# zhangxinsong-nlp/XFM

Hardware: AMD Instinct MI355X
Metric: image-text pairs/sec fwd+bwd, XFM-base 224px/30tok (higher is better)
Workload: dtype bf16; 1 GPU; Pretrain.py full multimodal step (ITC+ITM+MLM+MIM), XFM-base, synthetic 224px images + 30-token captions, random init; units_per_gpu=64, global_batch=64, dropout=True, ordered_reductions=True, grad_allreduce=False, parallelism=dp1, image_res=224

## Files before the change

### xfm_amd/csrc/gemm.hip

```cpp
#include "common.h"

enum { EPI_BF16 = 0, EPI_F32 = 1, EPI_GELU = 2, EPI_DGELU = 3, EPI_F32_ACC = 4 };

#define XFM_FENCE() asm volatile("" ::: "memory")
#define XFM_BAR()                    \
  do {                               \
    XFM_FENCE();                     \
    __builtin_amdgcn_s_barrier();    \
    XFM_FENCE();                     \
  } while (0)


struct GemmNT {
  const bf16* A; long lda;
  const bf16* B; long ldb;
  void* C; long ldc;
  const float* bias;
  bf16* aux; long ldaux;
  int M, N, K;
  int group_m;
  int k_splits;
  long split_stride;
#ifdef XFM_DIAG
  long long* dbg;
// ... 48 lines not shown
      for (int i = 0; i < 4; ++i) {
        v[i] = acc[mt][2 * np][i] + bv[i];
        v[4 + i] = acc[mt][2 * np + 1][i] + bv[4 + i];
      }
      const bool full = (nb + 8 <= g.N) && vec_c;
      if (EPI == EPI_F32 || EPI == EPI_F32_ACC) {
        float* cp = reinterpret_cast<float*>(g.C) + (long)m * g.ldc + nb;
        if (EPI == EPI_F32 && g.k_splits > 1) {
          cp += (long)blockIdx.y * g.split_stride;
        }
        if (EPI == EPI_F32_ACC && g.k_splits > 1) {
          for (int i = 0; i < 8; ++i)
            if (nb + i < g.N) atomicAdd(cp + i, v[i] - (blockIdx.y == 0 ? 0.f : bv[i]));
          continue;
        }
        if (EPI == EPI_F32_ACC) {
          for (int i = 0; i < 8; ++i)
            if (nb + i < g.N) v[i] += cp[i];
        }
        if (full) {
          *reinterpret_cast<f32x4*>(cp) = f32x4{v[0], v[1], v[2], v[3]};
          *reinterpret_cast<f32x4*>(cp + 4) = f32x4{v[4], v[5], v[6], v[7]};
        } else {
          for (int i = 0; i < 8; ++i)
            if (nb + i < g.N) cp[i] = v[i];
        }
      } else {
        bf16* cp = reinterpret_cast<bf16*>(g.C) + (long)m * g.ldc + nb;
        bf16x8 o;
        if (EPI == EPI_GELU) {
          bf16* ap = g.aux + (long)m * g.ldaux + nb;
          bf16x8 dact;
#pragma unroll
          for (int i = 0; i < 8; ++i) {
            const float x = bf2f(f2bf(v[i]));
            float cdf, pdf;
            gelu_parts(x, cdf, pdf);
            o[i] = f2bf(x * cdf);
            dact[i] = f2bf(fmaf(x, pdf, cdf));
          }
          if (full) *reinterpret_cast<bf16x8*>(ap) = dact;
          else
            for (int i = 0; i < 8; ++i)
              if (nb + i < g.N) ap[i] = dact[i];
        } else if (EPI == EPI_DGELU) {
          const bf16* ap = g.aux + (long)m * g.ldaux + nb;
          if (full && vec_aux) {
            const bf16x8 dact = pre_all[np][mt];
#pragma unroll
            for (int i = 0; i < 8; ++i) o[i] = f2bf(v[i] * bf2f(dact[i]));
          } else {
            for (int i = 0; i < 8; ++i) o[i] = (nb + i < g.N) ? f2bf(v[i] * bf2f(ap[i])) : f2bf(0.f);
          }
        } else {
#pragma unroll
          for (int i = 0; i < 8; ++i) o[i] = f2bf(v[i]);
        }
        if (full) *reinterpret_cast<bf16x8*>(cp) = o;
        else
          for (int i = 0; i < 8; ++i)
            if (nb + i < g.N) cp[i] = o[i];
      }
    }
  }
}


template <int BM, int BN, int EPI, int NS>
__global__ __launch_bounds__(256) void gemm_nt_kernel(GemmNT g) {
  constexpr int MT = BM / 32, NT = BN / 32;
  constexpr int LOADS = (BM + BN) / 32;
  constexpr int A_BYTES = BM * 128, B_BYTES = BN * 128, STAGE = A_BYTES + B_BYTES;
  extern __shared__ __attribute__((aligned(16))) char smem[];
  const int tid = threadIdx.x, lane = tid & 63, w = tid >> 6;
  const int wm = w >> 1, wn = w & 1;
  const int lr = lane & 15, lg = lane >> 4;
  const int tiles_n = (g.N + BN - 1) / BN, tiles_m = (g.M + BM - 1) / BM;
  const int wg = xcd_remap(blockIdx.x, gridDim.x);
  int tm, tn;
  grouped_tile(wg, tiles_m, tiles_n, g.group_m, tm, tn);
  const int m0 = tm * BM, n0 = tn * BN;

  const int nk_all = g.K / 64;
  const int nk_per = (nk_all + g.k_splits - 1) / g.k_splits;
  const int kt0 = blockIdx.y * nk_per;
  const int nk = nk_all - kt0 < nk_per ? nk_all - kt0 : nk_per;
  if (nk <= 0) return;
  auto stage = [&](int buf, int kt) {
    char* sA = smem + buf * STAGE;
    char* sB = sA + A_BYTES;
    const int k0 = (kt0 + kt) * 64;
#pragma unroll
    for (int i = 0; i < BM / 32; ++i) {
      const int blk = i * 4 + w;
      const int r = blk * 8 + (lane >> 3);
      const int c = (lane & 7) ^ swz_x(r);
      int gr = m0 + r;
      gr = gr < g.M ? gr : g.M - 1;
      const bf16* src = g.A + (long)gr * g.lda + k0 + c * 8;
      __builtin_amdgcn_global_load_lds(GLB_PTR(void, src), LDS_PTR(void, sA + blk * 1024), 16, 0, 0);
    }
#pragma unroll
    for (int i = 0; i < BN / 32; ++i) {
      const int blk = i * 4 + w;
      const int r = blk * 8 + (lane >> 3);
      const int c = (lane & 7) ^ swz_w(r);
      int gr = n0 + r;
      gr = gr < g.N ? gr : g.N - 1;
      const bf16* src = g.B + (long)gr * g.ldb + k0 + c * 8;
      __builtin_amdgcn_global_load_lds(GLB_PTR(void, src), LDS_PTR(void, sB + blk * 1024), 16, 0, 0);
    }
  };

  f32x4 acc[MT][NT];
#pragma unroll
  for (int i = 0; i < MT; ++i)
#pragma unroll
    for (int j = 0; j < NT; ++j) acc[i][j] = f32x4{0.f, 0.f, 0.f, 0.f};

  int xrow[MT], wrow[NT];
#pragma unroll
  for (int mt = 0; mt < MT; ++mt) xrow[mt] = wm * (BM / 2) + mt * 16 + lr;
#pragma unroll
  for (int nt = 0; nt < NT; ++nt) wrow[nt] = wn * (BN / 2) + (nt >> 1) * 32 + 8 * (lr >> 2) + 4 * (nt & 1) + (lr & 3);

  if (NS == 2) {
    stage(0, 0);
    asm volatile("s_waitcnt vmcnt(0)" ::: "memory");
    __syncthreads();
  } else {
#pragma unroll
    for (int s0 = 0; s0 < NS - 1; ++s0)
      if (s0 < nk) stage(s0, s0);
  }
  int slot = 0;
  for (int kt = 0; kt < nk; ++kt) {
    if (NS == 2) {
      if (kt + 1 < nk) stage((kt & 1) ^ 1, kt + 1);
    } else {
      const int younger = nk - 1 - kt < NS - 2 ? nk - 1 - kt : NS - 2;
      if (younger >= 2) asm volatile("s_waitcnt vmcnt(%0)" ::"n"(2 * LOADS) : "memory");
      else if (younger == 1) asm volatile("s_waitcnt vmcnt(%0)" ::"n"(LOADS) : "memory");
      else asm volatile("s_waitcnt vmcnt(0)" ::: "memory");
      XFM_BAR();
      if (kt + NS - 1 < nk) stage(slot == 0 ? NS - 1 : slot - 1, kt + NS - 1);
    }
    const int cur = NS == 2 ? (kt & 1) : slot;
    const char* sA = smem + cur * STAGE;
    const char* sB = sA + A_BYTES;
#pragma unroll
    for (int ks = 0; ks < 2; ++ks) {
      const int c = ks * 4 + lg;
      bf16x8 xf[MT], wf[NT];
#pragma unroll
      for (int mt = 0; mt < MT; ++mt)
        xf[mt] = *reinterpret_cast<const bf16x8*>(sA + xrow[mt] * 128 + ((c ^ swz_x(xrow[mt])) << 4));
#pragma unroll
      for (int nt = 0; nt < NT; ++nt)
        wf[nt] = *reinterpret_cast<const bf16x8*>(sB + wrow[nt] * 128 + ((c ^ swz_w(wrow[nt])) << 4));
#pragma unroll
      for (int mt = 0; mt < MT; ++mt)
#pragma unroll
        for (int nt = 0; nt < NT; ++nt)
          acc[mt][nt] = __builtin_amdgcn_mfma_f32_16x16x32_bf16(wf[nt], xf[mt], acc[mt][nt], 0, 0, 0);
    }
    if (NS == 2) {
      asm volatile("s_waitcnt vmcnt(0)" ::: "memory");
      __syncthreads();
    } else {
      slot = slot == NS - 1 ? 0 : slot + 1;
    }
  }

  gemm_epilogue<MT, NT, EPI>(g, acc, m0 + wm * (BM / 2), n0 + wn * (BN / 2), lr, lg);
}

template <int EPI>
__global__ __launch_bounds__(512) void gemm_nt_ring_kernel(GemmNT g) {
  constexpr int BM = 256, BN = 128, MT = 4, NT = 4;
  constexpr int A_BYTES = BM * 128, B_BYTES = BN * 128, STAGE = A_BYTES + B_BYTES;
  extern __shared__ __attribute__((aligned(16))) char smem[];
  const int tid = threadIdx.x, lane = tid & 63, w = tid >> 6;
  const int wm = w >> 1, wn = w & 1;
  const int lr = lane & 15, lg = lane >> 4;
  const int tiles_n = (g.N + BN - 1) / BN, tiles_m = (g.M + BM - 1) / BM;
  const int wg = xcd_remap(blockIdx.x, gridDim.x);
  int tm, tn;
  grouped_tile(wg, tiles_m, tiles_n, g.group_m, tm, tn);
  const int m0 = tm * BM, n0 = tn * BN;

  auto stage = [&](int slot, int kt) {
    char* sA = smem + slot * STAGE;
    char* sB = sA + A_BYTES;
    const int k0 = kt * 64;
#pragma unroll
    for (int i = 0; i < 4; ++i) {
      const int blk = i * 8 + w;
      const int r = blk * 8 + (lane >> 3);
      const int c = (lane & 7) ^ swz_x(r);
      int gr = m0 + r;
      gr = gr < g.M ? gr : g.M - 1;
      __builtin_amdgcn_global_load_lds(GLB_PTR(void, g.A + (long)gr * g.lda + k0 + c * 8), LDS_PTR(void, sA + blk * 1024), 16, 0, 0);
    }
#pragma unroll
    for (int i = 0; i < 2; ++i) {
      const int blk = i * 8 + w;
      const int r = blk * 8 + (lane >> 3);
      const int c = (lane & 7) ^ swz_w(r);
      int gr = n0 + r;
      gr = gr < g.N ? gr : g.N - 1;
      __builtin_amdgcn_global_load_lds(GLB_PTR(void, g.B + (long)gr * g.ldb + k0 + c * 8), LDS_PTR(void, sB + blk * 1024), 16, 0, 0);
    }
  };

  f32x4 acc[MT][NT];
#pragma unroll
  for (int i = 0; i < MT; ++i)
#pragma unroll
    for (int j = 0; j < NT; ++j) acc[i][j] = f32x4{0.f, 0.f, 0.f, 0.f};
  int xrow[MT], wrow[NT];
#pragma unroll
  for (int mt = 0; mt < MT; ++mt) xrow[mt] = wm * 64 + mt * 16 + lr;
#pragma unroll
  for (int nt = 0; nt < NT; ++nt) wrow[nt] = wn * 64 + (nt >> 1) * 32 + 8 * (lr >> 2) + 4 * (nt & 1) + (lr & 3);

  const int nk = g.K / 64;
  stage(0, 0);
  if (nk > 1) stage(1, 1);
  int slot = 0;
  for (int kt = 0; kt < nk; ++kt) {
    if (kt + 1 < nk) asm volatile("s_waitcnt vmcnt(6)" ::: "memory");
    else asm volatile("s_waitcnt vmcnt(0)" ::: "memory");
    __builtin_amdgcn_s_barrier();
    if (kt + 2 < nk) stage(slot == 0 ? 2 : slot - 1, kt + 2);
    const char* sA = smem + slot * STAGE;
    const char* sB = sA + A_BYTES;
#pragma unroll
    for (int ks = 0; ks < 2; ++ks) {
      const int c = ks * 4 + lg;
      bf16x8 xf[MT], wf[NT];
#pragma unroll
      for (int mt = 0; mt < MT; ++mt)
        xf[mt] = *reinterpret_cast<const bf16x8*>(sA + xrow[mt] * 128 + ((c ^ swz_x(xrow[mt])) << 4));
#pragma unroll
      for (int nt = 0; nt < NT; ++nt)
        wf[nt] = *reinterpret_cast<const bf16x8*>(sB + wrow[nt] * 128 + ((c ^ swz_w(wrow[nt])) << 4));
#pragma unroll
      for (int mt = 0; mt < MT; ++mt)
#pragma unroll
        for (int nt = 0; nt < NT; ++nt)
          acc[mt][nt] = __builtin_amdgcn_mfma_f32_16x16x32_bf16(wf[nt], xf[mt], acc[mt][nt], 0, 0, 0);
    }
    slot = slot == 2 ? 0 : slot + 1;
  }
  gemm_epilogue<MT, NT, EPI>(g, acc, m0 + wm * 64, n0 + wn * 64, lr, lg);
}

static int launch_nt_ring(const GemmNT& g, int epi, hipStream_t st) {
  const int tiles = cdiv(g.M, 256) * cdiv(g.N, 128);
  const size_t smem = 3 * (256 + 128) * 128;
#define XFM_RING_CASE(E)                                                                                       \
  case E: {                                                                                                    \
    static bool attr_set = false;                                                                              \
    if (!attr_set) {                                                                                           \
      (void)hipFuncSetAttribute(reinterpret_cast<const void*>(gemm_nt_ring_kernel<E>),                         \
                                hipFuncAttributeMaxDynamicSharedMemorySize, (int)smem);                        \
      attr_set = true;                                                                                         \
    }                                                                                                          \
    hipLaunchKernelGGL((gemm_nt_ring_kernel<E>), dim3(tiles), dim3(512), smem, st, g);                         \
    break;                                                                                                     \
  }
  switch (epi) {
    XFM_RING_CASE(EPI_BF16)
    XFM_RING_CASE(EPI_F32)
    XFM_RING_CASE(EPI_GELU)
    XFM_RING_CASE(EPI_DGELU)
    XFM_RING_CASE(EPI_F32_ACC)
    default:
      xfm_set_error("gemm_nt: bad epilogue %d", epi);
      return XFM_E_ARG;
  }
#undef XFM_RING_CASE
  return xfm_check_launch("gemm_nt_ring");
}

template <int J>
__device__ __forceinline__ int unit_row(int u) {
  if (J == 0) return u + (u & 64);
  if (J == 3) return u + 64 + (u & 64);
  if (J == 1) return ((u >> 5) << 6) + (u & 31);
  return ((u >> 5) << 6) + 32 + (u & 31);
}


__device__ __forceinline__ void wait_younger(int y) {
  if (y >= 3) asm volatile("s_waitcnt vmcnt(6)" ::: "memory");
  else if (y == 2) asm volatile("s_waitcnt vmcnt(4)" ::: "memory");
  else if (y == 1) asm volatile("s_waitcnt vmcnt(2)" ::: "memory");
  else asm volatile("s_waitcnt vmcnt(0)" ::: "memory");
}

template <int N>
__device__ __forceinline__ void wait_vm() { asm volatile("s_waitcnt vmcnt(%0)" ::"n"(N) : "memory"); }
template <int NS, int YMAX>
__device__ __forceinline__ void wait_units(int y) {
  if (YMAX >= 5 && y == 5) wait_vm<10 + NS>();
  else if (YMAX >= 4 && y == 4) wait_vm<8 + NS>();
  else if (y >= 3) wait_vm<6 + NS>();
  else if (y == 2) wait_vm<4 + NS>();
  else if (y == 1) wait_vm<2 + NS>();
  else wait_vm<NS>();
}
constexpr int NT256_D = 5;
template <int EPI, bool PERSIST>
__global__ __launch_bounds__(512) void gemm_nt_256_kernel(GemmNT g, int tiles) {
  constexpr int BM = 256, BN = 256, MT = 8, NT = 4;
  constexpr int D = NT256_D, R = D + 3, UNIT = 128 * 128;
  constexpr int NS = !PERSIST ? 0 : EPI == EPI_GELU || EPI == EPI_F32 ? 32 : EPI == EPI_F32_ACC ? 0 : 16;
  extern __shared__ __attribute__((aligned(16))) char smem[];
  const int tid = threadIdx.x, lane = tid & 63, w = __builtin_amdgcn_readfirstlane(tid >> 6);
  const int wr = w >> 2, wc = w & 3;
  const int lr = lane & 15, lg = lane >> 4;
  const int tiles_n = (g.N + BN - 1) / BN, tiles_m = (g.M + BM - 1) / BM;
  const int nk = g.K / 64;
  const int total = 4 * nk;

  unsigned soff[4][2];
  auto tile_origin = [&](int v, int& m0, int& n0) {
    int tm, tn;
    grouped_tile(xcd_remap(v, tiles), tiles_m, tiles_n, g.group_m, tm, tn);
    m0 = tm * BM;
    n0 = tn * BN;
  };
  auto tile_offsets = [&](int m0, int n0) {
#pragma unroll
    for (int i = 0; i < 2; ++i) {
      const int u = (i * 8 + w) * 8 + (lane >> 3);
      {
        const int r = unit_row<0>(u);
        int gr = m0 + r; gr = gr < g.M ? gr : g.M - 1;
        soff[0][i] = (unsigned)gr * (unsigned)g.lda + (((lane & 7) ^ swz_x(r)) << 3);
      }
      {
        const int r = unit_row<3>(u);
        int gr = m0 + r; gr = gr < g.M ? gr : g.M - 1;
        soff[3][i] = (unsigned)gr * (unsigned)g.lda + (((lane & 7) ^ swz_x(r)) << 3);
      }
      {
        const int r = unit_row<1>(u);
        int gr = n0 + r; gr = gr < g.N ? gr : g.N - 1;
        soff[1][i] = (unsigned)gr * (unsigned)g.ldb + (((lane & 7) ^ swz_w(r)) << 3);
      }
      {
        const int r = unit_row<2>(u);
        int gr = n0 + r; gr = gr < g.N ? gr : g.N - 1;
        soff[2][i] = (unsigned)gr * (unsigned)g.ldb + (((lane & 7) ^ swz_w(r)) << 3);
      }
    }
  };
  int iss = 0;
  auto issue = [&](int s) {
    char* base = smem + iss * UNIT + w * 1024;
    iss = iss + 1 == R ? 0 : iss + 1;
    if (s >= total) return;
    const int j = s & 3;
    const bf16* src = ((j == 0 || j == 3) ? g.A : g.B) + (s >> 2) * 64;
#pragma unroll
    for (int i = 0; i < 2; ++i) {
      const unsigned so = j == 0 ? soff[0][i] : j == 1 ? soff[1][i] : j == 2 ? soff[2][i] : soff[3][i];
      const unsigned lds_addr = (unsigned)(uintptr_t)LDS_PTR(void, base) + (unsigned)(i * 8192);
      asm volatile("s_mov_b32 m0, %1\n\ts_nop 0\n\tglobal_load_lds_dwordx4 %0, off" ::"v"(src + (size_t)so), "s"(lds_addr) : "memory", "m0");
    }
  };

  f32x4 acc[MT][NT];

  const int xs = swz_x(lr);
  const int wu = 8 * (lr >> 2) + (lr & 3);
  const int ws = swz_w(wu);
  const int xbase0 = (wr * 64 + lr) * 128 + (((0 + lg) ^ xs) << 4), xbase1 = (wr * 64 + lr) * 128 + (((4 + lg) ^ xs) << 4);
  const int wbase0 = (wc * 32 + wu) * 128 + (((0 + lg) ^ ws) << 4), wbase1 = (wc * 32 + wu) * 128 + (((4 + lg) ^ ws) << 4);

  bf16x8 xa[4][2], wb0[2][2], wb1[2][2];
  auto read_x = [&](const char* slot) {
#pragma unroll
    for (int m = 0; m < 4; ++m) {
      xa[m][0] = *reinterpret_cast<const bf16x8*>(slot + xbase0 + m * 2048);
      xa[m][1] = *reinterpret_cast<const bf16x8*>(slot + xbase1 + m * 2048);
    }
  };
  auto read_w = [&](const char* slot, bf16x8 (&wb)[2][2]) {
#pragma unroll
    for (int n = 0; n < 2; ++n) {
      wb[n][0] = *reinterpret_cast<const bf16x8*>(slot + wbase0 + n * 512);
      wb[n][1] = *reinterpret_cast<const bf16x8*>(slot + wbase1 + n * 512);
    }
  };
#define XFM_QUAD(MH, NH, WB)                                                                                     \
  do {                                                                                                           \
    __builtin_amdgcn_s_setprio(1);                                                                               \
    _Pragma("unroll") for (int ks = 0; ks < 2; ++ks)                                                             \
    _Pragma("unroll") for (int m = 0; m < 4; ++m)                                                                \
    _Pragma("unroll") for (int n = 0; n < 2; ++n)                                                                \
      acc[MH * 4 + m][NH * 2 + n] =                                                                              \
          __builtin_amdgcn_mfma_f32_16x16x32_bf16(WB[n][ks], xa[m][ks], acc[MH * 4 + m][NH * 2 + n], 0, 0, 0);  \
    __builtin_amdgcn_s_setprio(0);                                                                               \
  } while (0)

  int v = blockIdx.x, m0, n0;
  tile_origin(v, m0, n0);
  tile_offsets(m0, n0);
#pragma unroll
  for (int s = 0; s < D; ++s) issue(s);
  bool stores_behind = false;

#ifdef XFM_DIAG
  int dbg_n = 0;
#endif
  while (true) {
#ifdef XFM_DIAG
    if (g.dbg != nullptr && tid == 0) {
      long long* d = g.dbg + ((long)blockIdx.x * 8 + dbg_n) * 4;
      d[0] = v; d[1] = wall_clock64();
    }
#endif
#pragma unroll
    for (int i = 0; i < MT; ++i)
#pragma unroll
      for (int j = 0; j < NT; ++j) acc[i][j] = f32x4{0.f, 0.f, 0.f, 0.f};
    {
      const int y = (total - 1 < D - 1 ? total - 1 : D - 1) - 1;
      if (NS > 0 && stores_behind) wait_units<NS, D - 2>(y);
      else wait_units<0, D - 2>(y);
    }
    XFM_BAR();
    if (wr == 1) XFM_BAR();

    int rs = 0;
    for (int kt = 0; kt < nk; ++kt) {
      const int ph = 4 * kt;
      const bool plus = NS > 0 && stores_behind && kt == 0;
      const char* s_a0 = smem + rs * UNIT;
      const char* s_b0 = smem + (rs + 1 >= R ? rs + 1 - R : rs + 1) * UNIT;
      const char* s_b1 = smem + (rs + 2 >= R ? rs + 2 - R : rs + 2) * UNIT;
      const char* s_a1 = smem + (rs + 3 >= R ? rs + 3 - R : rs + 3) * UNIT;
      rs = rs + 4 >= R ? rs + 4 - R : rs + 4;
      int last;
      issue(ph + D);
      read_x(s_a0);
      read_w(s_b0, wb0);
      last = ph + D < total ? ph + D : total - 1;
      if (plus) wait_units<NS, D - 2>(last - (ph + 2));
      else wait_units<0, D - 2>(last - (ph + 2));
      XFM_BAR();
      XFM_QUAD(0, 0, wb0);
      XFM_BAR();
      issue(ph + D + 1);
      read_w(s_b1, wb1);
      last = ph + D + 1 < total ? ph + D + 1 : total - 1;
      if (plus) wait_units<NS, D - 2>(last - (ph + 3));
      else wait_units<0, D - 2>(last - (ph + 3));
      XFM_BAR();
      XFM_QUAD(0, 1, wb1);
      XFM_BAR();
      issue(ph + D + 2);
      read_x(s_a1);
      XFM_BAR();
      XFM_QUAD(1, 1, wb1);
      XFM_BAR();
      issue(ph + D + 3);
      last = ph + D + 3 < total ? ph + D + 3 : total - 1;
      wait_units<0, D - 2>(last - (ph + 5) < 0 ? 0 : last - (ph + 5));
      XFM_BAR();
      XFM_QUAD(1, 0, wb0);
      XFM_BAR();
    }
    if (wr == 0) XFM_BAR();
#ifdef XFM_DIAG
    if (g.dbg != nullptr && tid == 0) g.dbg[((long)blockIdx.x * 8 + dbg_n) * 4 + 2] = wall_clock64();
#endif
    const int cm0 = m0, cn0 = n0;
    float* lds_bias = reinterpret_cast<float*>(smem + (R - 1) * UNIT + w * 256);
    if (g.bias != nullptr) {
      int col = cn0 + wc * 64 + lane;
      col = col < g.N ? col : g.N - 1;
      const unsigned lds_addr = (unsigned)(uintptr_t)LDS_PTR(void, lds_bias);
      asm volatile("s_mov_b32 m0, %1\n\ts_nop 0\n\tglobal_load_lds_dword %0, off" ::"v"(g.bias + col), "s"(lds_addr) : "memory", "m0");
    } else {
      lds_bias[lane] = 0.f;
    }
    v += gridDim.x;
    const bool more = PERSIST && v < tiles;
    int ahead = 0;
    if (more) {
      tile_origin(v, m0, n0);
      tile_offsets(m0, n0);
      iss = 0;
#pragma unroll
      for (int s = 0; s < D; ++s) issue(s);
      ahead = total < D ? total : D;
    }
    wait_units<0, D>(ahead);
    if (g.bias == nullptr) asm volatile("s_waitcnt lgkmcnt(0)" ::: "memory");
    gemm_epilogue<MT, NT, EPI>(g, acc, cm0 + wr * 128, cn0 + wc * 64, lr, lg, lds_bias);
#ifdef XFM_DIAG
    if (g.dbg != nullptr && tid == 0) {
      g.dbg[((long)blockIdx.x * 8 + dbg_n) * 4 + 3] = wall_clock64();
      dbg_n = dbg_n < 7 ? dbg_n + 1 : 7;
    }
#endif
    if (!more) break;
    XFM_FENCE();
    stores_behind = cm0 + BM <= g.M && cn0 + BN <= g.N && (g.ldc % 8) == 0 && (EPI != EPI_GELU || (g.ldaux % 8) == 0);
  }
#undef XFM_QUAD
}

#ifdef XFM_DIAG
static XfmTimeline nt256_timeline = {nullptr, 0, 0};
#endif

template <int E, bool P>
static void launch_nt_256_as(const GemmNT& g, int grid, int tiles, hipStream_t st) {
  constexpr int smem = (NT256_D + 3) * 128 * 128;
  static bool attr_set = false;
  if (!attr_set) {
    (void)hipFuncSetAttribute(reinterpret_cast<const void*>(gemm_nt_256_kernel<E, P>), hipFuncAttributeMaxDynamicSharedMemorySize, smem);
    attr_set = true;
  }
  hipLaunchKernelGGL((gemm_nt_256_kernel<E, P>), dim3(grid), dim3(512), smem, st, g, tiles);
}

static int launch_nt_256(const GemmNT& g_in, int epi, hipStream_t st) {
  GemmNT g = g_in;
  const int tiles = cdiv(g.M, 256) * cdiv(g.N, 256);
  if ((unsigned long)g.M * (unsigned long)g.lda >= (1ul << 32) || (unsigned long)g.N * (unsigned long)g.ldb >= (1ul << 32)) {
    xfm_set_error("gemm_nt: operand too large for the 256x256 kernel's 32-bit element offsets");
    return XFM_E_ARG;
  }
  static const int persist_env = xfm_env_int("XFM_GEMM_PERSIST", 1);
  static const int cus = xfm_cu_count();
  const bool persist = persist_env && cus >= 8 && tiles > cus;
  const int grid = persist ? cus & ~7 : tiles;
#ifdef XFM_DIAG
  g.dbg = nt256_timeline.ptr;
  if (g.dbg != nullptr && nt256_timeline.bytes < (size_t)grid * XFM_NT256_STAMP_BYTES) {
    xfm_set_error("gemm_nt_256: timeline buffer of %zu bytes is short of %d workgroups x %d: launched without stamps", nt256_timeline.bytes, grid,
                  XFM_NT256_STAMP_BYTES);
    g.dbg = nullptr;
  }
#endif
#define XFM_256_CASE(E)                                            \
  case E:                                                          \
    if (persist) launch_nt_256_as<E, true>(g, grid, tiles, st);    \
    else launch_nt_256_as<E, false>(g, grid, tiles, st);           \
    break;
  switch (epi) {
    XFM_256_CASE(EPI_BF16)
    XFM_256_CASE(EPI_F32)
    XFM_256_CASE(EPI_GELU)
    XFM_256_CASE(EPI_DGELU)
    XFM_256_CASE(EPI_F32_ACC)
    default:
      xfm_set_error("gemm_nt: bad epilogue %d", epi);
      return XFM_E_ARG;
  }
#undef XFM_256_CASE
  return xfm_check_launch("gemm_nt_256");
}

template <int BM, int BN, int NS>
static int launch_nt(const GemmNT& g, int epi, hipStream_t st) {
  const int tiles = cdiv(g.M, BM) * cdiv(g.N, BN);
  const size_t smem = NS * (BM + BN) * 128;
#define XFM_NT_CASE(E)                                                                                         \
  case E: {                                                                                                    \
    static bool attr_set = false;                                                                              \
    if (!attr_set) {                                                                                           \
      (void)hipFuncSetAttribute(reinterpret_cast<const void*>(gemm_nt_kernel<BM, BN, E, NS>),                  \
                                hipFuncAttributeMaxDynamicSharedMemorySize, (int)smem);                        \
      attr_set = true;                                                                                         \
    }                                                                                                          \
    hipLaunchKernelGGL((gemm_nt_kernel<BM, BN, E, NS>), dim3(tiles, g.k_splits), dim3(256), smem, st, g);      \
    break;                                                                                                     \
  }
  switch (epi) {
    XFM_NT_CASE(EPI_BF16)
    XFM_NT_CASE(EPI_F32)
    XFM_NT_CASE(EPI_GELU)
    XFM_NT_CASE(EPI_DGELU)
    XFM_NT_CASE(EPI_F32_ACC)
    default:
      xfm_set_error("gemm_nt: bad epilogue %d", epi);
      return XFM_E_ARG;
  }
#undef XFM_NT_CASE
  return xfm_check_launch("gemm_nt");
}

static int nt_plan(int M, int N, int K, int epi, int tile_hint, int* rows_a_out, int* k_splits_out) {
  *rows_a_out = 0;
  *k_splits_out = 1;
  int cfg = tile_hint;
  if (cfg <= 0) {
    static const int split_env = xfm_env_int("XFM_GEMM_TAIL_SPLIT", 35);
    const long tn256 = cdiv(N, 256), t256 = (long)cdiv(M, 256) * tn256;
    if (split_env && tile_hint == 0 && M >= 2048 && t256 > 256 && t256 % 256 != 0 && (t256 % 256) * 100 < split_env * 256) {
      const int rows_a = (int)((t256 / 256) * 256 / tn256) * 256;
      if (rows_a > 0 && rows_a < M) {
        *rows_a_out = rows_a;
        return 5;
      }
    }
    if (M >= 2048 && (t256 >= 180 || (t256 >= 120 && M >= 8192))) cfg = 5;
    else if (M >= 2048 && t256 >= 120) cfg = 1;
    else if ((long)cdiv(M, 256) * cdiv(N, 128) >= 768) cfg = 4;
    else if ((long)cdiv(M, 128) * cdiv(N, 128) >= 800) cfg = 1;
    else if ((long)cdiv(M, 64) * cdiv(N, 128) >= 512) cfg = 2;
    else if (K >= 1536 && epi != EPI_F32_ACC && (long)cdiv(M, 64) * cdiv(N, 128) < 300) {
      cfg = 8;
    }
    else if ((long)cdiv(M, 64) * cdiv(N, 128) >= 128 || K >= 1536) {
      cfg = 7;
      const long t = (long)cdiv(M, 64) * cdiv(N, 128);
      if (epi == EPI_F32_ACC && K >= 8192 && t < 192) {
        int sp = (int)(512 / t);
        if (sp > K / 1024) sp = K / 1024;
        *k_splits_out = sp < 1 ? 1 : sp;
      }
    }
    else cfg = 3;
  }
  return cfg;
}

static GemmNT gemm_nt_args(const void* A, long lda, const void* B, long ldb, void* C, long ldc, const float* bias, int M, int N, int K) {
  static const int gm_env = xfm_env_int("XFM_GEMM_GROUP_M", 0);
  GemmNT g{};
  g.A = (const bf16*)A; g.lda = lda;
  g.B = (const bf16*)B; g.ldb = ldb;
  g.C = C; g.ldc = ldc;
  g.bias = bias;
  g.M = M; g.N = N; g.K = K;
  g.group_m = gm_env > 0 ? gm_env : 8;
  g.k_splits = 1;
  return g;
}

int xfm_gemm_nt_impl(const void* A, long lda, const void* B, long ldb, void* C, long ldc, const float* bias,
                     void* aux, long ldaux, int M, int N, int K, int epi, int tile_hint, hipStream_t st) {
  XFM_REQUIRE(M > 0 && N > 0 && K > 0, "gemm_nt: empty problem M=%d N=%d K=%d", M, N, K);
  XFM_REQUIRE(K % 64 == 0, "gemm_nt: K=%d must be a multiple of 64", K);
  XFM_REQUIRE(lda % 8 == 0 && ldb % 8 == 0, "gemm_nt: lda=%ld ldb=%ld must be multiples of 8", lda, ldb);
  XFM_REQUIRE(((uintptr_t)A % 16) == 0 && ((uintptr_t)B % 16) == 0 && ((uintptr_t)C % 16) == 0,
              "gemm_nt: operands must be 16-byte aligned");
  XFM_REQUIRE((epi != EPI_GELU && epi != EPI_DGELU) || aux != nullptr, "gemm_nt: epilogue %d needs aux", epi);
  GemmNT g = gemm_nt_args(A, lda, B, ldb, C, ldc, bias, M, N, K);
  g.aux = (bf16*)aux; g.ldaux = ldaux;
  int rows_a = 0, k_splits = 1;
  const int cfg = nt_plan(M, N, K, epi, tile_hint, &rows_a, &k_splits);
  if (rows_a > 0) {
    int rc = xfm_gemm_nt_impl(A, lda, B, ldb, C, ldc, bias, aux, ldaux, rows_a, N, K, epi, 5, st);
    if (rc != XFM_OK) return rc;
    const long esz = (epi == EPI_F32 || epi == EPI_F32_ACC) ? 4 : 2;
    return xfm_gemm_nt_impl((const bf16*)A + (long)rows_a * lda, lda, B, ldb, (char*)C + (long)rows_a * ldc * esz, ldc, bias,
                            aux ? (void*)((bf16*)aux + (long)rows_a * ldaux) : nullptr, ldaux, M - rows_a, N, K, epi, -1, st);
  }
  g.k_splits = k_splits;
  switch (cfg) {
    case 1: return launch_nt<128, 128, 2>(g, epi, st);
    case 2: return launch_nt<64, 128, 2>(g, epi, st);
    case 7: return launch_nt<64, 128, 3>(g, epi, st);
    case 8: return launch_nt<64, 64, 4>(g, epi, st);
    case 4: return launch_nt_ring(g, epi, st);
    case 5: return launch_nt_256(g, epi, st);
    default: return launch_nt<64, 64, 2>(g, epi, st);
  }
}

__global__ __launch_bounds__(256) void ksplit_reduce_kernel(const float* __restrict__ ws, int slices, long plane, int M, int N, void* __restrict__ out,
                                                            long ldo, int out_bf16) {
  const long e = ((long)blockIdx.x * 256 + threadIdx.x) * 8;
  if (e >= (long)M * N) return;
  const int m = (int)(e / N), n = (int)(e - (long)m * N);
  f32x4 a0 = *reinterpret_cast<const f32x4*>(ws + e), a1 = *reinterpret_cast<const f32x4*>(ws + e + 4);
  for (int s = 1; s < slices; ++s) {
    a0 += *reinterpret_cast<const f32x4*>(ws + (long)s * plane + e);
    a1 += *reinterpret_cast<const f32x4*>(ws + (long)s * plane + e + 4);
  }
  if (out_bf16) {
    bf16x8 o;
#pragma unroll
    for (int i = 0; i < 4; ++i) { o[i] = f2bf(a0[i]); o[4 + i] = f2bf(a1[i]); }
    *reinterpret_cast<bf16x8*>(reinterpret_cast<bf16*>(out) + (long)m * ldo + n) = o;
  } else {
    float* op = reinterpret_cast<float*>(out) + (long)m * ldo + n;
    *reinterpret_cast<f32x4*>(op) = a0;
    *reinterpret_cast<f32x4*>(op + 4) = a1;
  }
}

static int ksplit_plan(int M, int N, int K, int* nk_per_out) {
  const long t = (long)cdiv(M, 64) * cdiv(N, 128);
  int sp = 1;
  if (K >= 8192 && t < 192) {
    sp = (int)(512 / t);
    if (sp > K / 1024) sp = K / 1024;
    if (sp < 1) sp = 1;
  }
  const int nk_all = K / 64, nk_per = cdiv(nk_all, sp);
  *nk_per_out = nk_per;
  return cdiv(nk_all, nk_per);
}

long xfm_gemm_nt_ksplit_workspace_impl(int M, int N, int K) {
  if (M <= 0 || N <= 0 || K <= 0) return 0;
  int nk_per;
  const int slices = ksplit_plan(M, N, K, &nk_per);
  return slices > 1 ? (long)slices * M * N * 4 : 0;
}

int xfm_gemm_nt_ksplit_impl(const void* A, long lda, const void* B, long ldb, void* out, long ldo, int out_bf16, const float* bias, int M, int N,
                            int K, float* ws, long ws_bytes, hipStream_t st) {
  XFM_REQUIRE(M > 0 && N > 0 && K > 0 && K % 64 == 0, "gemm_nt_ksplit: bad shape M=%d N=%d K=%d", M, N, K);
  int nk_per;
  const int slices = ksplit_plan(M, N, K, &nk_per);
  if (slices <= 1) return xfm_gemm_nt_impl(A, lda, B, ldb, out, ldo, bias, nullptr, 0, M, N, K, out_bf16 ? EPI_BF16 : EPI_F32, 0, st);
  XFM_REQUIRE(N % 8 == 0 && ldo % 8 == 0 && ((uintptr_t)out % 16) == 0, "gemm_nt_ksplit: N=%d, ldo=%ld must be multiples of 8 and out 16-byte aligned", N, ldo);
  XFM_REQUIRE(lda % 8 == 0 && ldb % 8 == 0 && ((uintptr_t)A % 16) == 0 && ((uintptr_t)B % 16) == 0, "gemm_nt_ksplit: operands must be 16-byte aligned rows");
  XFM_REQUIRE(ws != nullptr && ((uintptr_t)ws % 16) == 0 && ws_bytes >= (long)slices * M * N * 4,
              "gemm_nt_ksplit: workspace of %ld bytes needed (xfm_gemm_nt_ksplit_workspace)", (long)slices * M * N * 4);
  GemmNT g = gemm_nt_args(A, lda, B, ldb, ws, (long)N, bias, M, N, K);
  g.k_splits = slices;
  g.split_stride = (long)M * N;
  XFM_REQUIRE(cdiv(K / 64, cdiv(K / 64, slices)) == slices, "gemm_nt_ksplit: slice plan mismatch");
  int rc = launch_nt<64, 128, 3>(g, EPI_F32, st);
  if (rc != XFM_OK) return rc;
  hipLaunchKernelGGL(ksplit_reduce_kernel, dim3(cdiv((long)M * N / 8, 256)), dim3(256), 0, st, ws, slices, (long)M * N, M, N, out, ldo, out_bf16);
  return xfm_check_launch("ksplit_reduce");
}

struct GemmTN {
  const bf16* dY; long ldy;
  const bf16* X; long ldx;
  float* dW; long ldw;
  float* dbias;
  int M, N, K;
  int m_per_split;
  float* ws;
  int direct;
};

#define TN_BATCH_MAX 4
struct TnBatch {
  int nb;
  int wg_per;
  long ws_stride;
  const bf16* dY[TN_BATCH_MAX];
  const bf16* X[TN_BATCH_MAX];
  float* dW[TN_BATCH_MAX];
  float* dbias[TN_BATCH_MAX];
};

__device__ __forceinline__ int swz_t(int r) { return ((r & 3) | (((r >> 3) & 1) << 2)) << 1; }

__device__ __forceinline__ bf16x8 tr_read_pair(const char* tile, int row0, int col0, int lr) {
  const int r = row0 + (lr >> 2);
  const int col = col0 + 4 * (lr & 3);
  const int off0 = r * 256 + ((((col >> 3)) ^ swz_t(r)) << 4) + (col & 7) * 2;
  const int r2 = r + 4;
  const int off1 = r2 * 256 + ((((col >> 3)) ^ swz_t(r2)) << 4) + (col & 7) * 2;
  const s16x4 lo = __builtin_amdgcn_ds_read_tr16_b64_v4i16(LDS_PTR(s16x4, tile + off0));
  const s16x4 hi = __builtin_amdgcn_ds_read_tr16_b64_v4i16(LDS_PTR(s16x4, tile + off1));
  union { struct { s16x4 a, b; } s; bf16x8 v; } u;
  u.s.a = lo;
  u.s.b = hi;
  return u.v;
}

__global__ __launch_bounds__(256) void gemm_tn_kernel(GemmTN g) {
  constexpr int TILE = 64 * 256;
  extern __shared__ __attribute__((aligned(16))) char smem[];
  const int tid = threadIdx.x, lane = tid & 63, w = tid >> 6;
  const int wn = w >> 1, wk = w & 1;
  const int lr = lane & 15, lg = lane >> 4;
  const int tiles_k = (g.K + 127) / 128, tiles_n = (g.N + 127) / 128;
  const int per_split = tiles_k * tiles_n;
  const int wg = xcd_remap(blockIdx.x, gridDim.x);
  const int split = wg / per_split, t = wg % per_split;
  const int n0 = (t / tiles_k) * 128, k0 = (t % tiles_k) * 128;
  const int mbeg = split * g.m_per_split;
  int mend = mbeg + g.m_per_split;
  mend = mend < g.M ? mend : g.M;
  const int nsteps = (mend - mbeg + 63) / 64;

  const bool do_bias = g.dbias != nullptr && k0 == 0;
  float bsum[8] = {0.f, 0.f, 0.f, 0.f, 0.f, 0.f, 0.f, 0.f};
  u32x4 ry[4], rx[4];
  auto gload = [&](int step) {
    const int mb = mbeg + step * 64;
#pragma unroll
    for (int i = 0; i < 4; ++i) {
      const int q = i * 256 + tid, r = q >> 4, c = q & 15;
      const int m = mb + r;
      const bool okm = m < mend;
      const int nn = n0 + c * 8, kk = k0 + c * 8;
      ry[i] = u32x4{0, 0, 0, 0};
      rx[i] = u32x4{0, 0, 0, 0};
      if (okm && nn < g.N) {
        if (nn + 8 <= g.N) ry[i] = *reinterpret_cast<const u32x4*>(g.dY + (long)m * g.ldy + nn);
        else {
          union { bf16 h[8]; u32x4 v; } u; u.v = u32x4{0, 0, 0, 0};
          for (int e = 0; e < 8; ++e) if (nn + e < g.N) u.h[e] = g.dY[(long)m * g.ldy + nn + e];
          ry[i] = u.v;
        }
      }
      if (okm && kk < g.K) rx[i] = *reinterpret_cast<const u32x4*>(g.X + (long)m * g.ldx + kk);
    }
  };
  auto lstore = [&](int buf) {
    char* sY = smem + buf * 2 * TILE;
    char* sX = sY + TILE;
#pragma unroll
    for (int i = 0; i < 4; ++i) {
      const int q = i * 256 + tid, r = q >> 4, c = q & 15;
      const int off = r * 256 + ((c ^ swz_t(r)) << 4);
      *reinterpret_cast<u32x4*>(sY + off) = ry[i];
// ... 984 lines not shown
```

Baseline: 1746 pairs/s.

## Deepen persistent NT256 GEMM prefetch ring across tile boundaries

For the persistent 256x256 NT GEMM, the LDS ring grows from 8 to 10 units and the next tile prefetches H=R-1 units ahead instead of D. This hides more of the next tile's global-load latency behind the current tile's epilogue. Steady-state issue stays D ahead, so the extra units are consumed at the start of each tile, and the wait logic is generalized to handle them. The cost is more LDS per block (160KB) and more complex vmcnt bookkeeping, with a risk of miscounted waits.

After: 1711 pairs/s. 2.0% lower.

```diff
diff --git a/xfm_amd/csrc/gemm.hip b/xfm_amd/csrc/gemm.hip
--- a/xfm_amd/csrc/gemm.hip
+++ b/xfm_amd/csrc/gemm.hip
@@ -374,20 +374,34 @@
 
 template <int N>
 __device__ __forceinline__ void wait_vm() { asm volatile("s_waitcnt vmcnt(%0)" ::"n"(N) : "memory"); }
+template <int NS, int Y, int YMAX>
+__device__ __forceinline__ void wait_units_above(int y) {
+  if constexpr (Y < YMAX) {
+    if (y == Y) wait_vm<2 * Y + NS>();
+    else wait_units_above<NS, Y + 1, YMAX>(y);
+  } else {
+    wait_vm<2 * YMAX + NS>();
+  }
+}
 template <int NS, int YMAX>
 __device__ __forceinline__ void wait_units(int y) {
-  if (YMAX >= 5 && y == 5) wait_vm<10 + NS>();
-  else if (YMAX >= 4 && y == 4) wait_vm<8 + NS>();
-  else if (y >= 3) wait_vm<6 + NS>();
-  else if (y == 2) wait_vm<4 + NS>();
-  else if (y == 1) wait_vm<2 + NS>();
-  else wait_vm<NS>();
+  static_assert(YMAX >= 3 && 2 * YMAX + NS <= 63, "vmcnt is a 6-bit field");
+  if (YMAX == 3 || y <= 3) {
+    if (y >= 3) wait_vm<6 + NS>();
+    else if (y == 2) wait_vm<4 + NS>();
+    else if (y == 1) wait_vm<2 + NS>();
+    else wait_vm<NS>();
+  } else {
+    wait_units_above<NS, 4, YMAX>(y);
+  }
 }
 constexpr int NT256_D = 5;
+constexpr int nt256_ring(bool persist) { return persist ? 10 : NT256_D + 3; }
 template <int EPI, bool PERSIST>
 __global__ __launch_bounds__(512) void gemm_nt_256_kernel(GemmNT g, int tiles) {
   constexpr int BM = 256, BN = 256, MT = 8, NT = 4;
-  constexpr int D = NT256_D, R = D + 3, UNIT = 128 * 128;
+  constexpr int D = NT256_D, R = nt256_ring(PERSIST), UNIT = 128 * 128;
+  constexpr int H = PERSIST ? R - 1 : D;
   constexpr int NS = !PERSIST ? 0 : EPI == EPI_GELU || EPI == EPI_F32 ? 32 : EPI == EPI_F32_ACC ? 0 : 16;
   extern __shared__ __attribute__((aligned(16))) char smem[];
   const int tid = threadIdx.x, lane = tid & 63, w = __builtin_amdgcn_readfirstlane(tid >> 6);
@@ -483,8 +497,13 @@
   tile_origin(v, m0, n0);
   tile_offsets(m0, n0);
 #pragma unroll
-  for (int s = 0; s < D; ++s) issue(s);
+  for (int s = 0; s < H; ++s) issue(s);
   bool stores_behind = false;
+  auto retire = [&](int x, int issued) {
+    const int y = (issued < total ? issued : total - 1) - x;
+    if (NS > 0 && stores_behind && x < H) wait_units<NS, H - 2>(y);
+    else wait_units<0, H - 2>(y);
+  };
 
 #ifdef XFM_DIAG
   int dbg_n = 0;
@@ -500,49 +519,39 @@
     for (int i = 0; i < MT; ++i)
 #pragma unroll
       for (int j = 0; j < NT; ++j) acc[i][j] = f32x4{0.f, 0.f, 0.f, 0.f};
-    {
-      const int y = (total - 1 < D - 1 ? total - 1 : D - 1) - 1;
-      if (NS > 0 && stores_behind) wait_units<NS, D - 2>(y);
-      else wait_units<0, D - 2>(y);
-    }
+    retire(1, H - 1);
     XFM_BAR();
     if (wr == 1) XFM_BAR();
 
     int rs = 0;
     for (int kt = 0; kt < nk; ++kt) {
       const int ph = 4 * kt;
-      const bool plus = NS > 0 && stores_behind && kt == 0;
       const char* s_a0 = smem + rs * UNIT;
       const char* s_b0 = smem + (rs + 1 >= R ? rs + 1 - R : rs + 1) * UNIT;
       const char* s_b1 = smem + (rs + 2 >= R ? rs + 2 - R : rs + 2) * UNIT;
       const char* s_a1 = smem + (rs + 3 >= R ? rs + 3 - R : rs + 3) * UNIT;
       rs = rs + 4 >= R ? rs + 4 - R : rs + 4;
-      int last;
-      issue(ph + D);
+      const bool i0 = H == D || ph + D >= H, i1 = H == D || ph + D + 1 >= H, i2 = H == D || ph + D + 2 >= H, i3 = H == D || ph + D + 3 >= H;
+      if (i0) issue(ph + D);
       read_x(s_a0);
       read_w(s_b0, wb0);
-      last = ph + D < total ? ph + D : total - 1;
-      if (plus) wait_units<NS, D - 2>(last - (ph + 2));
-      else wait_units<0, D - 2>(last - (ph + 2));
+      retire(ph + 2, i0 ? ph + D : H - 1);
       XFM_BAR();
       XFM_QUAD(0, 0, wb0);
       XFM_BAR();
-      issue(ph + D + 1);
+      if (i1) issue(ph + D + 1);
       read_w(s_b1, wb1);
-      last = ph + D + 1 < total ? ph + D + 1 : total - 1;
-      if (plus) wait_units<NS, D - 2>(last - (ph + 3));
-      else wait_units<0, D - 2>(last - (ph + 3));
+      retire(ph + 3, i1 ? ph + D + 1 : H - 1);
       XFM_BAR();
       XFM_QUAD(0, 1, wb1);
       XFM_BAR();
-      issue(ph + D + 2);
+      if (i2) issue(ph + D + 2);
       read_x(s_a1);
       XFM_BAR();
       XFM_QUAD(1, 1, wb1);
       XFM_BAR();
-      issue(ph + D + 3);
-      last = ph + D + 3 < total ? ph + D + 3 : total - 1;
-      wait_units<0, D - 2>(last - (ph + 5) < 0 ? 0 : last - (ph + 5));
+      if (i3) issue(ph + D + 3);
+      retire(ph + 5, i3 ? ph + D + 3 : H - 1);
       XFM_BAR();
       XFM_QUAD(1, 0, wb0);
       XFM_BAR();
@@ -569,10 +578,10 @@
       tile_offsets(m0, n0);
       iss = 0;
 #pragma unroll
-      for (int s = 0; s < D; ++s) issue(s);
-      ahead = total < D ? total : D;
-    }
-    wait_units<0, D>(ahead);
+      for (int s = 0; s < H; ++s) issue(s);
+      ahead = total < H ? total : H;
+    }
+    wait_units<0, H>(ahead);
     if (g.bias == nullptr) asm volatile("s_waitcnt lgkmcnt(0)" ::: "memory");
     gemm_epilogue<MT, NT, EPI>(g, acc, cm0 + wr * 128, cn0 + wc * 64, lr, lg, lds_bias);
 #ifdef XFM_DIAG
@@ -594,7 +603,7 @@
 
 template <int E, bool P>
 static void launch_nt_256_as(const GemmNT& g, int grid, int tiles, hipStream_t st) {
-  constexpr int smem = (NT256_D + 3) * 128 * 128;
+  constexpr int smem = nt256_ring(P) * 128 * 128;
   static bool attr_set = false;
   if (!attr_set) {
     (void)hipFuncSetAttribute(reinterpret_cast<const void*>(gemm_nt_256_kernel<E, P>), hipFuncAttributeMaxDynamicSharedMemorySize, smem);
```
